# unum-cloud/usearch

Measured on NVIDIA H100. Metric: QPS @ recall@10>=0.95, higher is better.
Workload: dtype f32

## Files before the change

### include/usearch_b200.h

```cpp
#ifndef USEARCH_B200_H
#define USEARCH_B200_H

#include <stdbool.h>
#include <stddef.h>
#include <stdint.h>

#ifdef __cplusplus
extern "C" {
#endif


typedef void* usearch_index_t;
typedef uint64_t usearch_key_t;
typedef float usearch_distance_t;
typedef char const* usearch_error_t;
typedef usearch_distance_t (*usearch_metric_t)(void const*, void const*);

typedef enum usearch_metric_kind_t {
    usearch_metric_unknown_k = 0,
    usearch_metric_cos_k = 1,
    usearch_metric_ip_k = 2,
    usearch_metric_l2sq_k = 3,
    usearch_metric_haversine_k = 4,
    usearch_metric_divergence_k = 5,
// ... 72 lines not shown
                           size_t* counts, usearch_error_t* error);


void usearch_add(usearch_index_t index, usearch_key_t key, void const* vector, usearch_scalar_kind_t vector_kind, usearch_error_t* error);
bool usearch_contains(usearch_index_t index, usearch_key_t key, usearch_error_t* error);
size_t usearch_count(usearch_index_t index, usearch_key_t key, usearch_error_t* error);
size_t usearch_get(usearch_index_t index, usearch_key_t key, size_t count, void* vector, usearch_scalar_kind_t vector_kind, usearch_error_t* error);
size_t usearch_remove(usearch_index_t index, usearch_key_t key, usearch_error_t* error);
size_t usearch_rename(usearch_index_t index, usearch_key_t from, usearch_key_t to, usearch_error_t* error);
usearch_distance_t usearch_distance(void const* vector_first, void const* vector_second, usearch_scalar_kind_t scalar_kind,
                                    size_t dimensions, usearch_metric_kind_t metric_kind, usearch_error_t* error);
void usearch_exact_search(void const* dataset, size_t dataset_size, size_t dataset_stride, void const* queries,
                          size_t queries_size, size_t queries_stride, usearch_scalar_kind_t scalar_kind, size_t dimensions,
                          usearch_metric_kind_t metric_kind, size_t count, size_t threads, usearch_key_t* keys,
                          size_t keys_stride, usearch_distance_t* distances, size_t distances_stride,
                          usearch_error_t* error);
void usearch_clear(usearch_index_t index, usearch_error_t* error);

void usearch_b200_add_many(usearch_index_t index, usearch_key_t const* keys, void const* vectors, size_t count,
                           size_t vectors_stride, usearch_scalar_kind_t vector_kind, usearch_error_t* error);
void usearch_b200_add_many_device(usearch_index_t index, usearch_key_t const* keys, void const* vectors, size_t count,
                                  size_t vectors_stride, usearch_scalar_kind_t vector_kind, usearch_error_t* error);

size_t usearch_b200_remove_many(usearch_index_t index, usearch_key_t const* keys, size_t count, bool compact,
                                size_t* pruned_edges, usearch_error_t* error);
size_t usearch_b200_count_many(usearch_index_t index, usearch_key_t const* keys, size_t count, size_t* counts,
                               usearch_error_t* error);
void usearch_b200_change_reuse_removed(usearch_index_t index, bool reuse, usearch_error_t* error);
bool usearch_b200_reuse_removed(usearch_index_t index);

size_t usearch_b200_join(usearch_index_t a, usearch_index_t b, size_t max_proposals, bool exact, usearch_key_t* a_keys_out,
                         usearch_key_t* b_keys_out, size_t capacity, size_t* stats4_out, usearch_error_t* error);
void usearch_b200_last_join_ms(usearch_index_t index, float* out3);
void usearch_b200_pairwise_distances(usearch_index_t index, usearch_key_t const* left_keys, usearch_key_t const* right_keys, size_t n,
                                     usearch_distance_t* out, usearch_error_t* error);


void usearch_b200_shards_unique_id(void* unique_id128, usearch_error_t* error);
void usearch_b200_shards_join(usearch_index_t index, int rank, int world, void const* unique_id128, usearch_error_t* error);
size_t usearch_b200_sharded_search_many(usearch_index_t index, void const* queries, size_t queries_count, size_t queries_stride,
                                        usearch_scalar_kind_t query_kind, size_t count, usearch_key_t* keys,
                                        usearch_distance_t* distances, size_t* counts, usearch_error_t* error);
void usearch_b200_sharded_search_many_device(usearch_index_t index, void const* queries, size_t queries_count,
                                             size_t queries_stride, size_t count, usearch_key_t* keys,
                                             usearch_distance_t* distances, uint32_t* counts, uint32_t* computed_distances,
                                             uint32_t* visited_members, void* cuda_stream, usearch_error_t* error);
size_t usearch_b200_shards_payload_bytes(size_t queries_count, size_t count);
void usearch_b200_merge_topk(void const* payloads, int world, size_t queries_count, size_t count, usearch_key_t* keys,
                             usearch_distance_t* distances, uint32_t* counts, usearch_error_t* error);


void usearch_b200_search_many_device(usearch_index_t index, void const* queries, size_t queries_count,
                                     size_t queries_stride, size_t count, usearch_key_t* keys,
                                     usearch_distance_t* distances, uint32_t* counts, uint32_t* computed_distances,
                                     uint32_t* visited_members, void* cuda_stream, usearch_error_t* error);

void usearch_b200_search_many_enqueue(usearch_index_t index, void const* queries, size_t queries_count,
                                      size_t queries_stride, size_t count, usearch_key_t* keys,
                                      usearch_distance_t* distances, uint32_t* counts, uint32_t* computed_distances,
                                      uint32_t* visited_members, void* cuda_stream, usearch_error_t* error);
void usearch_b200_search_many_finish(usearch_index_t index, usearch_error_t* error);

size_t usearch_b200_search_many_stats(usearch_index_t index, void const* queries, size_t queries_count,
                                      size_t queries_stride, usearch_scalar_kind_t query_kind, size_t count,
                                      usearch_key_t* keys, usearch_distance_t* distances, size_t* counts,
                                      uint64_t* computed_distances, uint64_t* visited_members, usearch_error_t* error);

size_t usearch_b200_filtered_search_many(usearch_index_t index, void const* queries, size_t queries_count,
                                         size_t queries_stride, usearch_scalar_kind_t query_kind, size_t count,
                                         usearch_key_t const* allowed_keys, size_t allowed_count, usearch_key_t* keys,
                                         usearch_distance_t* distances, size_t* counts, uint64_t* computed_distances,
                                         uint64_t* visited_members, usearch_error_t* error);

void usearch_b200_cluster_many(usearch_index_t index, void const* queries, size_t queries_count, size_t queries_stride,
                               usearch_scalar_kind_t query_kind, size_t level, usearch_key_t* keys,
                               usearch_distance_t* distances, uint64_t* computed_distances, uint64_t* visited_members,
                               usearch_error_t* error);

size_t usearch_b200_exact_search_many(usearch_index_t index, void const* queries, size_t queries_count,
                                      size_t queries_stride, usearch_scalar_kind_t query_kind, size_t count,
                                      usearch_key_t* keys, usearch_distance_t* distances, size_t* counts,
                                      usearch_error_t* error);

void usearch_b200_profile_phases(usearch_index_t index, int enable, uint64_t* counters16);
int usearch_b200_tune(usearch_index_t index, char const* knob, int value);
int usearch_b200_launch_plan(usearch_index_t index, size_t count, uint64_t* out16, usearch_error_t* error);
int usearch_b200_device(usearch_index_t index);
uint64_t usearch_b200_kernel_launches(usearch_index_t index);
float usearch_b200_last_kernel_ms(usearch_index_t index);
size_t usearch_b200_bytes_per_vector(usearch_index_t index);
size_t usearch_b200_max_level(usearch_index_t index);

#ifdef __cplusplus
}
#endif
#endif
```

### usearch_b200/csrc/c_abi.cu

```cuda
#include <sys/mman.h>
#include <sys/stat.h>
#include <fcntl.h>
#include <unistd.h>

#include <cstdio>
#include <algorithm>
#include <cstring>
#include <new>
#include <utility>
#include <vector>

#include "../../include/usearch_b200.h"
#include "frozen_index.h"

using namespace usearch_b200;

namespace {

uint32_t metric_to_char(usearch_metric_kind_t kind) {
    switch (kind) {
    case usearch_metric_ip_k: return METRIC_IP;
    case usearch_metric_l2sq_k: return METRIC_L2SQ;
    case usearch_metric_cos_k: return METRIC_COS;
    case usearch_metric_haversine_k: return 'h';
// ... 474 lines not shown
    if (!m || !s) return set_error(error, "Unknown metric kind!");
    set_error(error, exact_search_free(dataset, dataset_size, dataset_stride, queries, queries_size, queries_stride, s, dimensions, m, count,
                                       keys, keys_stride, distances, distances_stride));
}

void usearch_b200_cluster_many(usearch_index_t index, void const* queries, size_t queries_count, size_t queries_stride,
                               usearch_scalar_kind_t query_kind, size_t level, usearch_key_t* keys, usearch_distance_t* distances,
                               uint64_t* computed_distances, uint64_t* visited_members, usearch_error_t* error) {
    frozen_index_t* ix = as_index(index);
    uint32_t qs = scalar_to_char(query_kind);
    if (!qs) return set_error(error, "Unknown scalar kind!");
    set_error(error, search_host_guarded(ix, queries, queries_count, queries_stride, qs, 1, keys, 8, distances, 4, nullptr, computed_distances,
                                     visited_members, nullptr, nullptr, 0, false, (int)std::min<size_t>(level, 0x7FFF)));
}

size_t usearch_b200_exact_search_many(usearch_index_t index, void const* queries, size_t queries_count, size_t queries_stride,
                                      usearch_scalar_kind_t query_kind, size_t count, usearch_key_t* keys, usearch_distance_t* distances,
                                      size_t* counts, usearch_error_t* error) {
    frozen_index_t* ix = as_index(index);
    uint32_t qs = scalar_to_char(query_kind);
    if (!qs) { set_error(error, "Unknown scalar kind!"); return 0; }
    if (char const* e = ix->exact_host(queries, queries_count, queries_stride, qs, count, keys, distances, counts)) {
        set_error(error, e);
        return 0;
    }
    size_t total = 0;
    if (counts)
        for (size_t i = 0; i < queries_count; ++i) total += counts[i];
    return total;
}


void usearch_b200_shards_unique_id(void* unique_id128, usearch_error_t* error) { set_error(error, shards_unique_id(unique_id128)); }

void usearch_b200_shards_join(usearch_index_t index, int rank, int world, void const* unique_id128, usearch_error_t* error) {
    frozen_index_t* ix = as_index(index);
    std::lock_guard<std::mutex> lock(ix->mutex);
    set_error(error, ix->join_shards(rank, world, unique_id128));
}

size_t usearch_b200_sharded_search_many(usearch_index_t index, void const* queries, size_t queries_count, size_t queries_stride,
                                        usearch_scalar_kind_t query_kind, size_t count, usearch_key_t* keys,
                                        usearch_distance_t* distances, size_t* counts, usearch_error_t* error) {
    frozen_index_t* ix = as_index(index);
    uint32_t qs = scalar_to_char(query_kind);
    if (!qs) { set_error(error, "Unknown scalar kind!"); return 0; }
    if (char const* e = ix->sharded_search_host(queries, queries_count, queries_stride, qs, count, keys, distances, counts)) {
        set_error(error, e);
        return 0;
    }
    size_t total = 0;
    if (counts)
        for (size_t i = 0; i < queries_count; ++i) total += counts[i];
    return total;
}

void usearch_b200_sharded_search_many_device(usearch_index_t index, void const* queries, size_t queries_count, size_t queries_stride,
                                             size_t count, usearch_key_t* keys, usearch_distance_t* distances, uint32_t* counts,
                                             uint32_t* computed_distances, uint32_t* visited_members, void* cuda_stream,
                                             usearch_error_t* error) {
    frozen_index_t* ix = as_index(index);
    std::lock_guard<std::mutex> lock(ix->mutex);
    if (char const* e = ix->ensure_context()) return set_error(error, e);
    cudaStream_t s = cuda_stream ? static_cast<cudaStream_t>(cuda_stream) : ix->stream;
    char const* e = ix->sharded_search_device(queries, queries_count, queries_stride, count, keys, distances, counts,
                                              computed_distances, visited_members, s);
    if (!e && !cuda_stream && cudaStreamSynchronize(s) != cudaSuccess) e = "CUDA failure: synchronize";
    set_error(error, e);
}

size_t usearch_b200_shards_payload_bytes(size_t queries_count, size_t count) { return shards_payload_bytes(queries_count, count); }

void usearch_b200_merge_topk(void const* payloads, int world, size_t queries_count, size_t count, usearch_key_t* keys,
                             usearch_distance_t* distances, uint32_t* counts, usearch_error_t* error) {
    set_error(error, shards_merge_host(payloads, world, queries_count, count, keys, distances, counts));
}

void usearch_clear(usearch_index_t index, usearch_error_t*) {
    frozen_index_t* ix = as_index(index);
    std::lock_guard<std::mutex> lock(ix->mutex);
    ix->release_device();
}

void usearch_b200_profile_phases(usearch_index_t index, int enable, uint64_t* counters16) {
    frozen_index_t* ix = as_index(index);
    std::lock_guard<std::mutex> lock(ix->mutex);
    if (counters16) {
        std::memset(counters16, 0, 128);
        if (ix->phase_cycles.ptr) cudaMemcpy(counters16, ix->phase_cycles.ptr, 128, cudaMemcpyDeviceToHost);
    }
    ix->profile_phases = enable != 0;
    if (ix->profile_phases && !ix->phase_cycles.reserve(16)) cudaMemset(ix->phase_cycles.ptr, 0, 128);
}

int usearch_b200_tune(usearch_index_t index, char const* knob, int value) {
    frozen_index_t* ix = as_index(index);
    std::lock_guard<std::mutex> lock(ix->mutex);
    if (!std::strcmp(knob, "stage_sets")) ix->tune.stage_sets = value;
    else if (!std::strcmp(knob, "warps_per_sm")) ix->tune.warps_per_sm = value;
    else if (!std::strcmp(knob, "prefilter")) ix->tune.prefilter = value;
    else if (!std::strcmp(knob, "heap_head")) ix->tune.heap_head = value;
    else return -1;
    return 0;
}

int usearch_b200_launch_plan(usearch_index_t index, size_t count, uint64_t* out16, usearch_error_t* error) {
    frozen_index_t* ix = as_index(index);
    std::lock_guard<std::mutex> lock(ix->mutex);
    char const* e = ix->ensure_context();
    if (!e && (!ix->loaded || ix->d.n == 0)) e = "An empty index has no launch plan";
    launch_plan_t pl;
    if (!e) e = ix->plan((uint32_t)count, 0, pl);
    set_error(error, e);
    if (e) return -1;
    uint64_t const visits = pl.visited_bitmap_words ? (pl.visit_log_cap ? 2u : 1u) : 0u;
    uint64_t const v[16] = {pl.stage_sets, pl.warps_per_sm_target, (uint64_t)pl.blocks, pl.smem_per_warp,
                            pl.heap_smem_cap, pl.heap_spill_cap, visits, pl.visited_cap,
                            pl.code_pass, pl.code_smem_stride, pl.qsplit_len, pl.prefilter ? 1u : 0u,
                            pl.off_heap - pl.off_stage};
    std::memcpy(out16, v, sizeof(v));
    return 0;
}

int usearch_b200_device(usearch_index_t index) { return as_index(index)->device; }
uint64_t usearch_b200_kernel_launches(usearch_index_t index) { return as_index(index)->kernel_launches; }
float usearch_b200_last_kernel_ms(usearch_index_t index) { return as_index(index)->last_kernel_ms; }
size_t usearch_b200_bytes_per_vector(usearch_index_t index) { return as_index(index)->d.bytes_per_vector; }
size_t usearch_b200_max_level(usearch_index_t index) { return (size_t)as_index(index)->d.max_level; }

}
```

### usearch_b200/csrc/device_index.h

```cpp
#pragma once
#include <cstddef>
#include <cstdint>

namespace usearch_b200 {

struct pf_record_t;

constexpr uint32_t EMPTY_SLOT = 0xFFFFFFFFu;
constexpr uint32_t SNAN_BITS = 0x7FA00000u;

enum : uint32_t {
    METRIC_IP = 'i', METRIC_COS = 'c', METRIC_L2SQ = 'e', METRIC_HAMMING = 'b',
    METRIC_TANIMOTO = 't', METRIC_SORENSEN = 's', METRIC_JACCARD = 'j',
};
enum : uint32_t { SCALAR_B1 = 1, SCALAR_BF16 = 4, SCALAR_F64 = 10, SCALAR_F32 = 11, SCALAR_F16 = 12, SCALAR_I8 = 23 };

struct device_index_t {
    uint8_t const* vectors = nullptr;
    uint64_t const* keys = nullptr;
    uint32_t const* nbr0 = nullptr;
    uint32_t const* upper_base = nullptr;
    uint32_t const* upper = nullptr;
    uint32_t const* deleted_bits = nullptr;
    float const* norms = nullptr;
    int8_t const* codes = nullptr;
    pf_record_t const* shadow = nullptr;
    uint32_t code_stride = 0;
    uint64_t vec_stride = 0;
    uint32_t n = 0;
    uint32_t m0 = 0, m0_stride = 0;
    uint32_t m = 0, m_stride = 0;
    uint32_t entry_slot = 0;
    int32_t max_level = 0;
    uint32_t dims = 0;
    uint32_t bytes_per_vector = 0;
    uint32_t chunks16 = 0;
    uint32_t metric = 0, scalar = 0;
};

struct cand_t {
    float d;
    uint32_t s;
};

enum : uint32_t { STATUS_OK = 0, STATUS_VISITED_OVERFLOW = 1, STATUS_HEAP_OVERFLOW = 2 };

struct search_args_t {
    uint8_t const* queries = nullptr;
    uint64_t query_stride = 0;
    uint32_t nq = 0;
    uint32_t const* query_list = nullptr;
    uint32_t k = 0, ef = 0;
    int32_t cluster_end_level = -1;
    uint8_t const* task_levels = nullptr;
    uint32_t* out_slots = nullptr;
    uint64_t* out_keys = nullptr;
    float* out_dists = nullptr;
    uint32_t* out_counts = nullptr;
    uint32_t* out_computed = nullptr;
    uint32_t* out_visited = nullptr;
    uint32_t* status = nullptr;
    uint32_t const* allow_bits = nullptr;
    uint32_t* work_counter = nullptr;
    uint32_t* visited = nullptr;
    uint32_t visited_cap = 0;
    uint32_t visited_bitmap_words = 0;
    uint32_t* visit_log = nullptr;
    uint32_t visit_log_cap = 0;
    cand_t* heap_spill = nullptr;
    uint32_t heap_spill_cap = 0;
    uint32_t heap_smem_cap = 0;
    uint32_t smem_per_warp = 0, off_top_d = 0, off_top_s = 0, off_cand_s = 0, off_cand_d = 0, off_heap = 0;
    uint32_t off_bars = 0, off_stage = 0, stage_stride = 0;
    uint32_t stage_sets = 1;
    uint32_t prefilter = 0, code_pass = 0, code_smem_stride = 0, off_surv_b2 = 0;
    uint32_t off_qsplit = 0, qsplit_len = 0;
    unsigned long long* phase_cycles = nullptr;
};

}
```

### usearch_b200/csrc/frozen_index.cu

```cuda
#include "cuda_check.h"
#include "f64_casts.h"
#include "frozen_index.h"
#include "prefilter_bound.h"

#include <algorithm>
#include <cmath>
#include <cstdlib>
#include <cstring>

namespace usearch_b200 {

namespace {

uint64_t rd_u64(uint8_t const* p) { uint64_t v; std::memcpy(&v, p, 8); return v; }
uint32_t rd_u32(uint8_t const* p) { uint32_t v; std::memcpy(&v, p, 4); return v; }
int16_t rd_i16(uint8_t const* p) { int16_t v; std::memcpy(&v, p, 2); return v; }
uint32_t ceil2(uint64_t v) { uint64_t r = 1; while (r < v) r <<= 1; return (uint32_t)std::min<uint64_t>(r, 1ull << 31); }
uint32_t round_up(uint32_t v, uint32_t m) { return (v + m - 1) / m * m; }


}

int default_device() {
    if (char const* dev = std::getenv("USEARCH_B200_DEVICE")) return std::atoi(dev);
// ... 470 lines not shown
    if (char const* e = work_counter.reserve(2)) return e;
    size_t const words = warps * pl.visited_words_per_warp();
    bool const grown = words > visited.capacity;
    if (char const* e = visited.reserve(words)) return e;
    if (grown) visited_zeroed_words = 0;
    if (pl.visit_log_cap) {
        if (char const* e = visit_log.reserve(warps * pl.visit_log_cap)) return e;
        if (visited_zeroed_words < words) {
            if (cudaMemsetAsync(visited.ptr, 0, words * 4, s) != cudaSuccess) return "CUDA failure: memset";
            visited_zeroed_words = words;
        }
    } else
        visited_zeroed_words = 0;
    if (char const* e = heap_spill.reserve(warps * pl.heap_spill_cap)) return e;
    a = search_args_t{};
    a.ef = pl.ef;
    a.work_counter = work_counter.ptr;
    a.visited = visited.ptr;
    a.visited_cap = pl.visited_cap;
    a.visited_bitmap_words = pl.visited_bitmap_words;
    a.visit_log = pl.visit_log_cap ? visit_log.ptr : nullptr;
    a.visit_log_cap = pl.visit_log_cap;
    a.heap_spill = heap_spill.ptr;
    a.heap_spill_cap = pl.heap_spill_cap;
    a.heap_smem_cap = pl.heap_smem_cap;
    a.smem_per_warp = pl.smem_per_warp;
    a.off_top_d = pl.off_top_d; a.off_top_s = pl.off_top_s; a.off_cand_s = pl.off_cand_s;
    a.off_cand_d = pl.off_cand_d; a.off_heap = pl.off_heap;
    a.off_bars = pl.off_bars; a.off_stage = pl.off_stage; a.stage_stride = pl.stage_stride;
    a.stage_sets = pl.stage_sets;
    a.prefilter = pl.prefilter ? 1u : 0u;
    a.code_pass = pl.code_pass;
    a.code_smem_stride = pl.code_smem_stride;
    a.off_surv_b2 = pl.off_surv_b2;
    a.off_qsplit = pl.off_qsplit; a.qsplit_len = pl.qsplit_len;
    return nullptr;
}

char const* frozen_index_t::search_device(void const* d_queries, size_t nq, size_t stride, size_t k, uint64_t* d_keys,
                                          float* d_dists, uint32_t* d_counts, uint32_t* d_computed, uint32_t* d_cycles,
                                          cudaStream_t s, bool defer) {
    if (nq == 0 || k == 0) return nullptr;
    if (nq > 0x7FFFFFFFull) return "Too many queries in one batch";
    if (char const* e = ensure_context()) return e;
    if (!loaded || d.n == 0) {
        CU(search_fill_empty(d_keys, d_dists, d_counts, d_computed, d_cycles, nq, k, s));
        return nullptr;
    }
    launch_plan_t pl;
    if (char const* e = plan((uint32_t)k, 0, pl)) return e;
    int const wpb = search_warps_per_block();
    int blocks = (int)std::min<size_t>((size_t)pl.blocks, (nq + wpb - 1) / wpb);
    size_t warps = (size_t)blocks * wpb;

    if (char const* e = h_status.reserve(nq)) return e;
    uint32_t* status_ptr = nullptr;
    if (defer) {
        if (pending_free.empty()) pending_free.emplace_back(new device_buffer_t<uint32_t>());
        device_buffer_t<uint32_t>* buf = pending_free.back();
        pending_free.pop_back();
        if (char const* e = buf->reserve(nq)) { pending_free.push_back(buf); return e; }
        pending.push_back(pending_search_t{buf, search_args_t{}, pl.maxed, s});
        status_ptr = buf->ptr;
    } else {
        if (char const* e = status.reserve(nq)) return e;
        status_ptr = status.ptr;
    }
    search_args_t a;
    if (char const* e = prepare_launch(pl, warps, a, s)) return e;
    a.queries = static_cast<uint8_t const*>(d_queries);
    a.query_stride = stride;
    a.nq = (uint32_t)nq;
    a.k = (uint32_t)k;
    a.out_keys = d_keys;
    a.out_dists = d_dists;
    a.out_counts = d_counts;
    a.out_computed = d_computed;
    a.out_visited = d_cycles;
    a.status = status_ptr;
    a.allow_bits = active_allow_bits;
    a.cluster_end_level = active_cluster_end_level;

    if (profile_phases) {
        if (char const* e = phase_cycles.reserve(16)) return e;
        a.phase_cycles = phase_cycles.ptr;
    }
    CU(cudaMemsetAsync(work_counter.ptr, 0, 8, s));
    CU(cudaEventRecord(ev_begin, s));
    CU(search_launch(d, a, blocks, pl.smem_per_block, s));
    CU(cudaEventRecord(ev_end, s));
    kernel_launches += 1;
    if (defer) {
        pending.back().args = a;
        return nullptr;
    }
    CU(cudaMemcpyAsync(h_status.ptr, status.ptr, nq * 4, cudaMemcpyDeviceToHost, s));
    CU(cudaStreamSynchronize(s));
    CU(cudaEventElapsedTime(&last_kernel_ms, ev_begin, ev_end));
    return retry_overflowed(a, pl.maxed, s);
}

char const* frozen_index_t::search_finish() {
    char const* first_error = nullptr;
    for (pending_search_t& p : pending) {
        char const* e = cuda_error(cudaStreamSynchronize(p.stream));
        if (!e) e = h_status.reserve(p.args.nq);
        if (!e) e = cuda_error(cudaMemcpy(h_status.ptr, p.status->ptr, (size_t)p.args.nq * 4, cudaMemcpyDeviceToHost));
        if (!e) e = retry_overflowed(p.args, p.maxed, p.stream);
        if (e && !first_error) first_error = e;
        pending_free.push_back(p.status);
    }
    pending.clear();
    if (ev_begin && ev_end && !first_error) cudaEventElapsedTime(&last_kernel_ms, ev_begin, ev_end);
    return first_error;
}

char const* frozen_index_t::retry_overflowed(search_args_t const& a, bool maxed, cudaStream_t s) {
    size_t const nq = a.nq, k = a.k;
    int const wpb = search_warps_per_block();
    std::vector<uint32_t> failed;
    for (size_t i = 0; i < nq; ++i)
        if (h_status.ptr[i] != STATUS_OK) failed.push_back((uint32_t)i);
    uint64_t scale = 1;
    while (!failed.empty()) {
        if (maxed) return "Search scratch overflow that full-size scratch could not fix";
        scale *= 8;
        launch_plan_t rp;
        if (char const* e = plan((uint32_t)k, (uint32_t)std::min<uint64_t>(scale, 1u << 30), rp)) return e;
        maxed = rp.maxed;
        size_t const bytes_per_warp = (size_t)rp.visited_words_per_warp() * 4 + (size_t)rp.heap_spill_cap * 8;
        size_t max_warps = std::max<size_t>(wpb, ((size_t)2 << 30) / bytes_per_warp / wpb * wpb);
        int rblocks = (int)std::min<size_t>({(size_t)rp.blocks, (failed.size() + wpb - 1) / wpb, max_warps / wpb});
        rblocks = std::max(rblocks, 1);
        size_t rwarps = (size_t)rblocks * wpb;
        if (char const* e = retry_list.reserve(failed.size())) return e;
        CU(cudaMemcpyAsync(retry_list.ptr, failed.data(), failed.size() * 4, cudaMemcpyHostToDevice, s));
        search_args_t r;
        if (char const* e = prepare_launch(rp, rwarps, r, s)) return e;
        r.queries = a.queries; r.query_stride = a.query_stride; r.k = a.k;
        r.out_keys = a.out_keys; r.out_dists = a.out_dists; r.out_counts = a.out_counts;
        r.out_computed = a.out_computed; r.out_visited = a.out_visited; r.status = a.status;
        r.allow_bits = a.allow_bits; r.cluster_end_level = a.cluster_end_level; r.phase_cycles = a.phase_cycles;
        r.nq = (uint32_t)failed.size();
        r.query_list = retry_list.ptr;
        CU(cudaMemsetAsync(work_counter.ptr, 0, 8, s));
        CU(search_launch(d, r, rblocks, rp.smem_per_block, s));
        kernel_launches += 1;
        CU(cudaMemcpyAsync(h_status.ptr, a.status, nq * 4, cudaMemcpyDeviceToHost, s));
        CU(cudaStreamSynchronize(s));
        std::vector<uint32_t> still;
        for (uint32_t qi : failed)
            if (h_status.ptr[qi] != STATUS_OK) still.push_back(qi);
        failed.swap(still);
    }
    return nullptr;
}


namespace {

uint16_t f32_to_f16_rn(float f) {
    uint32_t x;
    std::memcpy(&x, &f, 4);
    uint32_t sign = (x >> 16) & 0x8000u;
    uint32_t mant = x & 0x7FFFFFu;
    int32_t exp = (int32_t)((x >> 23) & 0xFF);
    if (exp == 255) return (uint16_t)(sign | 0x7C00u | (mant ? 0x200u | (mant >> 13) : 0));
// ... 419 lines not shown
```

### usearch_b200/csrc/search_kernel.cu

```cuda
#include <cuda_runtime.h>

#include <cstdlib>

#include "device_index.h"
#include "metrics.cuh"
#include "warp_primitives.cuh"

namespace usearch_b200 {

constexpr int THREADS = 32;
constexpr int LOADS_IN_FLIGHT = 8;
constexpr int BATCH_LOADS = 4;

__device__ __forceinline__ uint32_t hash_slot(uint32_t s) { return s * 0x9E3779B1u; }


struct heap_t {
    uint32_t smem_addr;
    cand_t* spill;
    uint32_t smem_cap;
    static __device__ __forceinline__ cand_t lds(uint32_t addr) {
        cand_t c;
        asm volatile("ld.shared.v2.b32 {%0, %1}, [%2];" : "=f"(c.d), "=r"(c.s) : "r"(addr));
        return c;
// ... 310 lines not shown
        if ((uint32_t)lane < ncand) w.cand_d[lane] = M::finalize(w.cand_d[lane], qc, n0);
        if ((uint32_t)lane + 32 < ncand) w.cand_d[lane + 32] = M::finalize(w.cand_d[lane + 32], qc, n1);
        for (uint32_t c = 64 + lane; c < ncand; c += 32) w.cand_d[c] = M::finalize(w.cand_d[c], qc, __ldg(ix.norms + w.cand_s[c]));
        __syncwarp();
    }
}

__device__ __forceinline__ pf_record_t ldg_record(pf_record_t const* p) {
    float4 const v = __ldg(reinterpret_cast<float4 const*>(p));
    return pf_record_t{v.x, v.y, v.z, v.w};
}

__device__ __forceinline__ double warp_sum_f64(double v) {
#pragma unroll
    for (int o = 16; o; o >>= 1) v += __shfl_xor_sync(0xffffffffu, v, o);
    return v;
}

__device__ __forceinline__ double warp_max_f64(double v) {
#pragma unroll
    for (int o = 16; o; o >>= 1) v = fmax(v, __shfl_xor_sync(0xffffffffu, v, o));
    return v;
}

__device__ __forceinline__ uint32_t qsplit_word_place(uint32_t word) { return (word & ~7u) + (word & 3u) * 2u + ((word >> 2) & 1u); }

__device__ __forceinline__ pf_query_split_t split_query(float const* qa, uint32_t n, uint8_t* q1, uint8_t* q2, uint32_t len,
                                                        int lane) {
    double mx1 = 0.0;
    bool finite = true;
    for (uint32_t i = (uint32_t)lane; i < n; i += 32) {
        double const x = fabs((double)qa[i]);
        finite = finite && x < INFINITY;
        mx1 = fmax(mx1, x);
    }
    mx1 = warp_max_f64(mx1);
    finite = __all_sync(0xffffffffu, finite);
    float const sa1 = pf_scale(mx1);
    bool const usable = finite && sa1 > 0.0f;
    double mx2 = 0.0;
    int8_t c1, c2;
    if (usable)
        for (uint32_t i = (uint32_t)lane; i < n; i += 32) mx2 = fmax(mx2, fabs(pf_split_step((double)qa[i], sa1, c1)));
    mx2 = warp_max_f64(mx2);
    float const sa2 = usable ? pf_scale(mx2) : 0.0f;
    double e2 = 0.0;
    for (uint32_t wd = (uint32_t)lane; wd < len / 4; wd += 32) {
        uint32_t p1 = 0, p2 = 0;
#pragma unroll
        for (uint32_t b = 0; b < 4; ++b) {
            uint32_t const i = 4 * wd + b;
            c1 = c2 = 0;
            if (usable && i < n) {
                double const r2 = pf_split_step(pf_split_step((double)qa[i], sa1, c1), sa2, c2);
                e2 += r2 * r2;
            }
            p1 |= (uint32_t)(uint8_t)c1 << (8 * b);
            p2 |= (uint32_t)(uint8_t)c2 << (8 * b);
        }
        reinterpret_cast<uint32_t*>(q1)[qsplit_word_place(wd)] = p1;
        reinterpret_cast<uint32_t*>(q2)[qsplit_word_place(wd)] = p2;
    }
    e2 = warp_sum_f64(e2);
    __syncwarp();
    return usable ? pf_query_split_t{sa1, sa2, pf_round_up_norm(e2)} : pf_query_split_t{0.0f, 0.0f, INFINITY};
}

__device__ __forceinline__ void ldmatrix_x4(uint32_t addr, uint32_t& r0, uint32_t& r1, uint32_t& r2, uint32_t& r3) {
    asm volatile("ldmatrix.sync.aligned.m8n8.x4.shared.b16 {%0, %1, %2, %3}, [%4];"
                 : "=r"(r0), "=r"(r1), "=r"(r2), "=r"(r3)
                 : "r"(addr));
}

__device__ __forceinline__ void imma_16832(int (&c)[4], uint32_t a0, uint32_t a1, uint32_t a2, uint32_t a3, uint32_t b0, uint32_t b1) {
    asm volatile("mma.sync.aligned.m16n8k32.row.col.s32.s8.s8.s32 {%0,%1,%2,%3}, {%4,%5,%6,%7}, {%8,%9}, {%0,%1,%2,%3};"
                 : "+r"(c[0]), "+r"(c[1]), "+r"(c[2]), "+r"(c[3])
                 : "r"(a0), "r"(a1), "r"(a2), "r"(a3), "r"(b0), "r"(b1));
}

template <class M>
__device__ __forceinline__ uint32_t measure_prefiltered(device_index_t const& ix, search_args_t const& a, warp_ctx_t& w,
                                                     typename M::qconst_t qc, pf_query_bound_t const& qb,
                                                     pf_query_split_t const& sp, float radius, uint32_t ncand, int lane) {
    constexpr uint32_t MAX_TILES = 4;
    uint8_t* const smem = reinterpret_cast<uint8_t*>(w.q4);
    float* const surv_b2 = reinterpret_cast<float*>(smem + a.off_surv_b2);
    uint32_t const cs = ix.code_stride, scs = a.code_smem_stride, ksteps = a.qsplit_len / 32;
    uint32_t const bar = w.bars_addr;
    uint32_t const g = (uint32_t)lane >> 2, sub = (uint32_t)lane & 3;
    uint32_t const b_addr = smem_u32(smem + a.off_qsplit) + g * a.qsplit_len + 8u * sub;
    uint32_t const a_addr = w.stage_addr + ((uint32_t)lane & 7u) * scs + (((uint32_t)lane >> 3) & 1u) * 8u * scs + ((uint32_t)lane >> 4) * 16u;
    double const sa1 = (double)sp.sa1, sa2 = (double)sp.sa2;
    uint32_t ns = 0;
    for (uint32_t base = 0; base < ncand; base += a.code_pass) {
        uint32_t const cnt = min(a.code_pass, ncand - base);
        if (lane == 0) mbar_expect_tx(bar, cnt * cs);
        __syncwarp();
        pf_record_t r0{}, r1{};
        uint32_t s0 = 0, s1 = 0;
        if ((uint32_t)lane < cnt) {
            s0 = w.cand_s[base + lane];
            bulk_copy_g2s(w.stage_addr + lane * scs, ix.codes + (size_t)s0 * cs, cs, bar);
            r0 = ldg_record(ix.shadow + s0);
        }
        if ((uint32_t)lane + 32 < cnt) {
            s1 = w.cand_s[base + lane + 32];
            bulk_copy_g2s(w.stage_addr + (lane + 32) * scs, ix.codes + (size_t)s1 * cs, cs, bar);
            r1 = ldg_record(ix.shadow + s1);
        }
        if (a.phase_cycles) {
            long long const t = clock64();
            mbar_wait(bar, w.phase & 1u);
            w.t_code += (uint32_t)(clock64() - t);
        } else
            mbar_wait(bar, w.phase & 1u);
        w.phase ^= 1u;
        long long const t_dot = a.phase_cycles ? clock64() : 0;
        uint32_t const ntiles = (cnt + 15) / 16;
        int acc[2][MAX_TILES][4] = {};
        uint32_t fa[2][MAX_TILES][4], fb[2][2];
        auto load = [&](uint32_t k, uint32_t(&A)[MAX_TILES][4], uint32_t(&B)[2]) {
            B[0] = B[1] = 0u;
            if (lane < 8) asm volatile("ld.shared.v2.b32 {%0, %1}, [%2];" : "=r"(B[0]), "=r"(B[1]) : "r"(b_addr + 32u * k));
#pragma unroll
            for (uint32_t t = 0; t < MAX_TILES; ++t)
                if (t < ntiles) ldmatrix_x4(a_addr + t * 16u * scs + 32u * k, A[t][0], A[t][1], A[t][2], A[t][3]);
        };
        auto mma = [&](int (&C)[MAX_TILES][4], uint32_t const(&A)[MAX_TILES][4], uint32_t const(&B)[2]) {
#pragma unroll
            for (uint32_t t = 0; t < MAX_TILES; ++t)
                if (t < ntiles) imma_16832(C[t], A[t][0], A[t][1], A[t][2], A[t][3], B[0], B[1]);
        };
        load(0, fa[0], fb[0]);
        uint32_t k = 0;
        for (; k + 2 <= ksteps; k += 2) {
            load(k + 1, fa[1], fb[1]);
            mma(acc[0], fa[0], fb[0]);
            if (k + 2 < ksteps) load(k + 2, fa[0], fb[0]);
            mma(acc[1], fa[1], fb[1]);
        }
        if (k < ksteps) mma(acc[0], fa[0], fb[0]);
#pragma unroll
        for (uint32_t t = 0; t < MAX_TILES; ++t) {
            uint32_t const i = 16u * t + g;
            int const d1 = acc[0][t][0] + acc[1][t][0], d2 = acc[0][t][1] + acc[1][t][1];
            int const d1h = acc[0][t][2] + acc[1][t][2], d2h = acc[0][t][3] + acc[1][t][3];
            if (sub == 0 && i < cnt) w.cand_d[base + i] = __double2float_rn(sa1 * (double)d1 + sa2 * (double)d2);
            if (sub == 0 && i + 8 < cnt) w.cand_d[base + i + 8] = __double2float_rn(sa1 * (double)d1h + sa2 * (double)d2h);
        }
        __syncwarp();
        long long const t_bound = a.phase_cycles ? clock64() : 0;
        if (a.phase_cycles) w.t_dot += (uint32_t)(t_bound - t_dot);
        uint32_t const lt = (1u << lane) - 1u;
#pragma unroll
        for (int h = 0; h < 2; ++h) {
            uint32_t const i = (uint32_t)lane + 32u * (uint32_t)h, c = base + i;
            if (32u * (uint32_t)h >= cnt) break;
            pf_record_t const r = h ? r1 : r0;
            bool keep = false;
            if (i < cnt) keep = !(M::pf_lower(w.cand_d[c], r, qb) >= (double)radius);
            uint32_t const bal = __ballot_sync(0xffffffffu, keep);
            if (keep) {
                w.cand_s[ns + __popc(bal & lt)] = h ? s1 : s0;
                surv_b2[ns + __popc(bal & lt)] = r.b2;
            }
            ns += __popc(bal);
        }
        __syncwarp();
        if (a.phase_cycles) w.t_bound += (uint32_t)(clock64() - t_bound);
    }
    if (ns) {
        measure_staged<M>(ix, a, w, qc, ns, lane, w.cand_s, w.cand_d);
        __syncwarp();
        if constexpr (M::NORMS) {
            for (uint32_t j = lane; j < ns; j += 32) w.cand_d[j] = M::finalize(w.cand_d[j], qc, surv_b2[j]);
            __syncwarp();
        }
    }
    return ns;
}

__device__ __forceinline__ bool slot_allowed(device_index_t const& ix, search_args_t const& a, uint32_t s) {
    if (ix.deleted_bits && ((ix.deleted_bits[s >> 5] >> (s & 31)) & 1u)) return false;
    if (a.allow_bits && !((a.allow_bits[s >> 5] >> (s & 31)) & 1u)) return false;
    return true;
}


template <class M, bool STAGED, bool INSERT>
__device__ __forceinline__ void search_one(device_index_t const& ix, search_args_t const& a, uint32_t qi, uint32_t out_row,
                                           int const bl_arg, warp_ctx_t& w, heap_t const& heap, uint32_t* visited, int lane) {
    uint32_t const k = a.k, ef = a.ef;
    constexpr bool insert = INSERT;
    int const bl = INSERT ? bl_arg : 0;
    uint32_t const width = bl == 0 ? ix.m0 : ix.m;
    auto row_of = [&](uint32_t slot) -> uint32_t const* {
        if (bl == 0) return ix.nbr0 + (size_t)slot * ix.m0_stride;
        uint32_t const ub = __ldg(ix.upper_base + slot);
        return ix.upper + ((size_t)ub + (uint32_t)(bl - 1)) * ix.m_stride;
    };
    uint32_t top_size = 0, heap_size = 0, computed = 0, cycles = 0, status = STATUS_OK;
    uint32_t visited_total = 0;
    bool log_overflow_out = false;
    bool const prof = a.phase_cycles != nullptr;
    uint32_t pc0 = 0, pc1 = 0, pc2 = 0, pc4 = 0, pc5 = 0, n_push = 0, max_heap = 0, n_pref = 0, n_surv = 0;
    constexpr bool PF = prefilter_of<M>::value && STAGED && !INSERT;
    long long tp = prof ? clock64() : 0;
    w.t_wait = 0;
    w.t_code = 0;
    w.t_dot = 0;
    w.t_bound = 0;
#define PHASE(acc)                                  \
    if (prof) {                                     \
        long long now_ = clock64();                 \
        acc += (uint32_t)(now_ - tp);               \
        tp = now_;                                  \
    }
    float* const top_d = w.top_d;
    uint32_t* const top_s = w.top_s;
    bool const topreg = ef <= 32u * TOP_E;
    float rtd[TOP_E];
    uint32_t rts[TOP_E];
#pragma unroll
    for (int c = 0; c < TOP_E; ++c) { rtd[c] = 0.f; rts[c] = 0u; }
    uint32_t* const cand_s = w.cand_s;
    float* const cand_d = w.cand_d;

    if (ix.n != 0 && k != 0) {
        {
            uint8_t const* src = a.queries + (size_t)qi * a.query_stride;
            uint32_t const bpv = ix.bytes_per_vector;
            bool wide = ((reinterpret_cast<size_t>(src) | a.query_stride) & 15) == 0 && a.query_stride >= (uint64_t)ix.chunks16 * 16;
            if (wide) {
                for (uint32_t j = lane; j < ix.chunks16; j += 32) w.q4[j] = reinterpret_cast<uint4 const*>(src)[j];
            } else {
                uint8_t* dst = reinterpret_cast<uint8_t*>(w.q4);
                for (uint32_t b = lane; b < ix.chunks16 * 16; b += 32) dst[b] = b < bpv ? src[b] : (uint8_t)0;
            }
        }
        bool const bitmap = a.visited_bitmap_words != 0;
        bool const logged = bitmap && a.visit_log != nullptr;
        uint32_t* const vlog = logged ? a.visit_log + (size_t)blockIdx.x * a.visit_log_cap : nullptr;
        bool log_overflow = false;
        if (!logged) {
            uint32_t const fill = bitmap ? 0u : EMPTY_SLOT;
            uint4 const word = make_uint4(fill, fill, fill, fill);
            uint4* v4 = reinterpret_cast<uint4*>(visited);
            uint32_t const n4 = (bitmap ? a.visited_bitmap_words : a.visited_cap) / 4;
            for (uint32_t j = lane; j < n4; j += 32) v4[j] = word;
        }
        __threadfence_block();
        __syncwarp();
        typename M::qconst_t qc = M::prepare(w.q4, ix.chunks16, lane);
        pf_query_split_t pf_sp{0.f, 0.f, INFINITY};
        pf_query_bound_t pf_qb{};
        if constexpr (PF) {
            if (a.prefilter) {
                float const a2 = cos_f32_t::self_dot(w.q4, ix.chunks16, lane);
                uint8_t* const q1 = reinterpret_cast<uint8_t*>(w.q4) + a.off_qsplit;
                pf_sp = split_query(reinterpret_cast<float const*>(w.q4), ix.dims, q1, q1 + a.qsplit_len, a.qsplit_len, lane);
                pf_qb = pf_query_bound(a2, ix.dims, pf_sp.rho_a);
            }
        }
        uint32_t const vmask = a.visited_cap - 1;
        uint32_t visited_count = 0;

        uint32_t closest = ix.entry_slot;
        if (lane == 0) cand_s[0] = closest;
        __syncwarp();
        measure_list<M, STAGED>(ix, a, w, qc, 1, lane);
        computed += 1;
        float closest_d = cand_d[0];
        __syncwarp();
        bool const cluster = a.cluster_end_level >= 0;
        int const end_level = cluster ? a.cluster_end_level : bl;
        for (int level = ix.max_level; level > end_level; --level) {
            bool changed;
            do {
                changed = false;
                uint32_t const ubase = ix.upper_base[closest];
                uint32_t const* row = ix.upper + ((size_t)ubase + (uint32_t)(level - 1)) * ix.m_stride;
                uint32_t n = 0;
                for (uint32_t b = 0; b < ix.m; b += 32) {
                    uint32_t i = b + lane;
                    uint32_t s = (i < ix.m && ubase != EMPTY_SLOT) ? row[i] : EMPTY_SLOT;
                    bool valid = s != EMPTY_SLOT;
                    uint32_t bal = __ballot_sync(0xffffffffu, valid);
                    if (valid) cand_s[n + __popc(bal & ((1u << lane) - 1))] = s;
                    n += __popc(bal);
                }
                __syncwarp();
                measure_list<M, STAGED>(ix, a, w, qc, n, lane);
                computed += n;
                for (uint32_t b = 0; b < n; b += 32) {
                    uint32_t i = b + lane;
                    float d = i < n ? cand_d[i] : 0.f;
                    bool better = i < n && d < closest_d;
                    float best = better ? d : __int_as_float(0x7f800000);
                    uint32_t best_i = better ? i : 0xFFFFFFFFu;
#pragma unroll
                    for (int o = 16; o; o >>= 1) {
                        float od = __shfl_xor_sync(0xffffffffu, best, o);
                        uint32_t oi = __shfl_xor_sync(0xffffffffu, best_i, o);
                        if (oi != 0xFFFFFFFFu && (best_i == 0xFFFFFFFFu || od < best || (od == best && oi < best_i))) {
                            best = od;
                            best_i = oi;
                        }
                    }
                    if (best_i != 0xFFFFFFFFu) {
                        closest_d = best;
                        closest = cand_s[best_i];
                        changed = true;
                    }
                }
                __syncwarp();
                cycles += 1;
            } while (changed);
        }

        if (lane == 0) cand_s[0] = closest;
        __syncwarp();
        measure_list<M, STAGED>(ix, a, w, qc, 1, lane);
        computed += 1;
        float radius = cand_d[0];
        __syncwarp();
        if (lane == 0 && !cluster) {
            heap.set_root(cand_t{radius, closest});
            if (bitmap) atomicOr(&visited[closest >> 5], 1u << (closest & 31));
            else atomicCAS(&visited[hash_slot(closest) & vmask], EMPTY_SLOT, closest);
            if (logged) vlog[0] = closest;
        }
        heap_size = cluster ? 0 : 1;
        visited_count = cluster ? 0 : 1;
        uint32_t pre_node = EMPTY_SLOT, pre_s0 = EMPTY_SLOT, pre_s1 = EMPTY_SLOT;
        constexpr bool WIDE = !STAGED;
        uint32_t pre_s2 = EMPTY_SLOT, pre_s3 = EMPTY_SLOT;
        PHASE(pc0)
        {
            bool allowed = cluster || (insert ? closest != qi : slot_allowed(ix, a, closest));
            if (allowed) {
                if (topreg) {
                    if (lane == 0) { rtd[0] = radius; rts[0] = closest; }
                } else if (lane == 0) { top_d[0] = radius; top_s[0] = closest; }
                top_size = 1;
            }
        }
        __syncwarp();

        while (heap_size) {
            cand_t cur = heap.root();
            if (cur.d > radius && top_size == ef) break;
            uint32_t const* row = row_of(cur.s);
            uint32_t s0, s1, s2 = EMPTY_SLOT, s3 = EMPTY_SLOT;
            if (cur.s == pre_node) {
                s0 = pre_s0;
                s1 = pre_s1;
                if constexpr (WIDE) { s2 = pre_s2; s3 = pre_s3; }
            } else {
                s0 = lane < (int)width ? __ldg(row + lane) : EMPTY_SLOT;
                s1 = lane + 32 < (int)width ? __ldg(row + lane + 32) : EMPTY_SLOT;
                if constexpr (WIDE) {
                    s2 = lane + 64 < (int)width ? __ldg(row + lane + 64) : EMPTY_SLOT;
                    s3 = lane + 96 < (int)width ? __ldg(row + lane + 96) : EMPTY_SLOT;
                }
            }
            __syncwarp();
            uint32_t o0 = 0xFFFFFFFFu, o1 = 0xFFFFFFFFu, o2 = 0xFFFFFFFFu, o3 = 0xFFFFFFFFu;
            if (bitmap) {
                if (s0 != EMPTY_SLOT) o0 = atomicOr(&visited[s0 >> 5], 1u << (s0 & 31));
                if (s1 != EMPTY_SLOT) o1 = atomicOr(&visited[s1 >> 5], 1u << (s1 & 31));
                if constexpr (WIDE) {
                    if (s2 != EMPTY_SLOT) o2 = atomicOr(&visited[s2 >> 5], 1u << (s2 & 31));
                    if (s3 != EMPTY_SLOT) o3 = atomicOr(&visited[s3 >> 5], 1u << (s3 & 31));
                }
            }
            if (!heap.template pop_warp<PF ? 16 : 8>(heap_size, lane)) {
                if (lane == 0) heap.pop(heap_size);
            }
            heap_size -= 1;
            cycles += 1;
            __syncwarp();
            if (heap_size) {
                pre_node = heap.root().s;
                uint32_t const* next_row = row_of(pre_node);
                pre_s0 = lane < (int)width ? __ldg(next_row + lane) : EMPTY_SLOT;
                pre_s1 = lane + 32 < (int)width ? __ldg(next_row + lane + 32) : EMPTY_SLOT;
                if constexpr (WIDE) {
                    pre_s2 = lane + 64 < (int)width ? __ldg(next_row + lane + 64) : EMPTY_SLOT;
                    pre_s3 = lane + 96 < (int)width ? __ldg(next_row + lane + 96) : EMPTY_SLOT;
                }
            } else
                pre_node = EMPTY_SLOT;
            PHASE(pc1)

            uint32_t ncand = 0;
            if (bitmap) {
                bool f0 = s0 != EMPTY_SLOT && !((o0 >> (s0 & 31)) & 1u);
                bool f1 = s1 != EMPTY_SLOT && !((o1 >> (s1 & 31)) & 1u);
                uint32_t bal0 = __ballot_sync(0xffffffffu, f0), bal1 = __ballot_sync(0xffffffffu, f1);
                uint32_t const lt = (1u << lane) - 1;
                if (f0) cand_s[__popc(bal0 & lt)] = s0;
// ... 456 lines not shown
```

### usearch_b200/index.py

```python
from __future__ import annotations

import ctypes as C
import os
from dataclasses import dataclass
from typing import Dict, Optional, Union

import numpy as np

HERE = os.path.dirname(os.path.abspath(__file__))
LIB_PATH = os.path.join(HERE, "libusearch_b200.so")

METRIC_KIND = {"cos": 1, "ip": 2, "l2sq": 3, "haversine": 4, "divergence": 5, "pearson": 6, "jaccard": 7,
               "hamming": 8, "tanimoto": 9, "sorensen": 10}
SCALAR_KIND = {"f32": 1, "f64": 2, "f16": 3, "i8": 4, "b1": 5, "bf16": 6}
_NP_TO_SCALAR = {np.dtype(np.float32): "f32", np.dtype(np.float64): "f64", np.dtype(np.float16): "f16",
                 np.dtype(np.int8): "i8", np.dtype(np.uint8): "b1"}
_BITS = {"f32": 32, "f64": 64, "f16": 16, "bf16": 16, "i8": 8, "b1": 1}


class _InitOptions(C.Structure):
    _fields_ = [("metric_kind", C.c_int), ("metric", C.c_void_p), ("quantization", C.c_int),
                ("dimensions", C.c_size_t), ("connectivity", C.c_size_t), ("expansion_add", C.c_size_t),
                ("expansion_search", C.c_size_t), ("multi", C.c_bool)]

# ... 459 lines not shown
            keys.ctypes.data_as(C.c_void_p), distances.ctypes.data_as(C.c_void_p),
            computed.ctypes.data_as(C.c_void_p) if stats else None, visited.ctypes.data_as(C.c_void_p) if stats else None,
            C.byref(err))
        _raise(err)
        if stats:
            self.last_computed, self.last_visited = computed, visited
        return keys, distances

    def search(self, vectors: np.ndarray, count: int = 10, *, stats: bool = False, threads: int = 0, exact: bool = False,
               log=False, progress=None, _allowed: Optional[np.ndarray] = None) -> Union[Matches, BatchMatches]:
        vectors = np.asarray(vectors)
        single = vectors.ndim == 1
        if single:
            vectors = vectors[None, :]
        if vectors.ndim != 2:
            raise ValueError("Expects a matrix or a vector")
        if not vectors.flags.c_contiguous and vectors.strides[1] != vectors.itemsize:
            vectors = np.ascontiguousarray(vectors)
        kind = self._kind_of(vectors)
        expect_cols = (self.ndim * _BITS[kind] + 7) // 8 // vectors.itemsize if kind != "b1" else (self.ndim + 7) // 8
        if vectors.shape[1] != expect_cols:
            raise ValueError("The number of columns must match the dimensionality of the index")
        nq = vectors.shape[0]
        keys = np.zeros((nq, count), dtype=np.uint64)
        distances = np.zeros((nq, count), dtype=np.float32)
        counts = np.zeros(nq, dtype=np.uint64)
        err = C.c_char_p()
        vm = cd = 0
        if exact:
            self._lib.usearch_b200_exact_search_many(
                self._h, vectors.ctypes.data_as(C.c_void_p), nq, vectors.strides[0], SCALAR_KIND[kind], count,
                keys.ctypes.data_as(C.c_void_p), distances.ctypes.data_as(C.c_void_p),
                counts.ctypes.data_as(C.c_void_p), C.byref(err))
            _raise(err)
        elif _allowed is not None:
            computed = np.zeros(nq, dtype=np.uint64)
            visited = np.zeros(nq, dtype=np.uint64)
            self._lib.usearch_b200_filtered_search_many(
                self._h, vectors.ctypes.data_as(C.c_void_p), nq, vectors.strides[0], SCALAR_KIND[kind], count,
                _allowed.ctypes.data_as(C.c_void_p), _allowed.size, keys.ctypes.data_as(C.c_void_p),
                distances.ctypes.data_as(C.c_void_p), counts.ctypes.data_as(C.c_void_p),
                computed.ctypes.data_as(C.c_void_p), visited.ctypes.data_as(C.c_void_p), C.byref(err))
            _raise(err)
            self.last_computed, self.last_visited = computed, visited
            vm, cd = int(visited.sum()), int(computed.sum())
        elif stats:
            computed = np.zeros(nq, dtype=np.uint64)
            visited = np.zeros(nq, dtype=np.uint64)
            self._lib.usearch_b200_search_many_stats(
                self._h, vectors.ctypes.data_as(C.c_void_p), nq, vectors.strides[0], SCALAR_KIND[kind], count,
                keys.ctypes.data_as(C.c_void_p), distances.ctypes.data_as(C.c_void_p),
                counts.ctypes.data_as(C.c_void_p), computed.ctypes.data_as(C.c_void_p),
                visited.ctypes.data_as(C.c_void_p), C.byref(err))
            _raise(err)
            self.last_computed, self.last_visited = computed, visited
            vm, cd = int(visited.sum()), int(computed.sum())
        else:
            self._lib.usearch_search_many(
                self._h, vectors.ctypes.data_as(C.c_void_p), nq, vectors.strides[0], SCALAR_KIND[kind], count,
                keys.ctypes.data_as(C.c_void_p), keys.strides[0], distances.ctypes.data_as(C.c_void_p),
                distances.strides[0], counts.ctypes.data_as(C.c_void_p), C.byref(err))
            _raise(err)
        if single:
            n = int(counts[0])
            return Matches(keys[0, :n], distances[0, :n], vm, cd)
        return BatchMatches(keys, distances, counts, vm, cd)

    def tune(self, **knobs: int) -> None:
        for name, value in knobs.items():
            if self._lib.usearch_b200_tune(self._h, name.encode(), int(value)) != 0:
                raise ValueError(f"unknown knob {name}")

    def launch_plan(self, count: int = 10) -> dict:
        out = np.zeros(16, dtype=np.uint64)
        err = C.c_char_p()
        self._lib.usearch_b200_launch_plan(self._h, int(count), out.ctypes.data_as(C.c_void_p), C.byref(err))
        _raise(err)
        plan = dict(zip(LAUNCH_PLAN_FIELDS, (int(v) for v in out)))
        plan["visits"] = _VISITS[plan["visits"]]
        plan["prefilter"] = bool(plan["prefilter"])
        return plan

    def profile_phases(self, enable: bool = True) -> dict:
        out = np.zeros(16, dtype=np.uint64)
        self._lib.usearch_b200_profile_phases(self._h, int(enable), out.ctypes.data_as(C.c_void_p))
        names = ["setup_descent", "heap_pop", "row_visited", "vector_wait", "distance_math", "accept", "output"]
        q = max(int(out[7]), 1)
        return {"queries": int(out[7]), **{n: float(out[i]) / q for i, n in enumerate(names)},
                "pushes": float(out[8]) / q, "avg_max_heap": float(out[9]) / q, "max_heap": int(out[10]),
                "prefiltered": float(out[11]) / q, "survivors": float(out[12]) / q, "code_wait": float(out[13]) / q,
                "prefilter_dot": float(out[14]) / q, "prefilter_bound": float(out[15]) / q,
                "survivor_math": float(out[4] - out[14] - out[15]) / q}

    def join_shards(self, rank: int, world: int, unique_id: bytes) -> None:
        err = C.c_char_p()
        buf = (C.c_char * 128).from_buffer_copy(unique_id)
        self._lib.usearch_b200_shards_join(self._h, rank, world, buf, C.byref(err))
        _raise(err)

    def sharded_search(self, vectors: np.ndarray, count: int = 10) -> BatchMatches:
        vectors = np.ascontiguousarray(vectors)
        if vectors.ndim == 1:
            vectors = vectors[None, :]
        kind = self._kind_of(vectors)
        nq = vectors.shape[0]
        keys = np.zeros((nq, count), dtype=np.uint64)
        distances = np.zeros((nq, count), dtype=np.float32)
        counts = np.zeros(nq, dtype=np.uint64)
        err = C.c_char_p()
        self._lib.usearch_b200_sharded_search_many(self._h, vectors.ctypes.data_as(C.c_void_p), nq, vectors.strides[0],
                                                   SCALAR_KIND[kind], count, keys.ctypes.data_as(C.c_void_p),
                                                   distances.ctypes.data_as(C.c_void_p), counts.ctypes.data_as(C.c_void_p),
                                                   C.byref(err))
        _raise(err)
        return BatchMatches(keys, distances, counts)

    def sharded_search_device(self, queries_ptr: int, nq: int, stride: int, count: int, keys_ptr: int, distances_ptr: int,
                              counts_ptr: int, computed_ptr: int = 0, visited_ptr: int = 0, stream: int = 0) -> None:
        err = C.c_char_p()
        self._lib.usearch_b200_sharded_search_many_device(self._h, queries_ptr, nq, stride, count, keys_ptr, distances_ptr,
                                                          counts_ptr, computed_ptr or None, visited_ptr or None,
                                                          stream or None, C.byref(err))
        _raise(err)

    def search_enqueue(self, queries_ptr: int, nq: int, stride: int, count: int, keys_ptr: int, distances_ptr: int,
                       counts_ptr: int, computed_ptr: int = 0, visited_ptr: int = 0, stream: int = 0) -> None:
        err = C.c_char_p()
        self._lib.usearch_b200_search_many_enqueue(self._h, queries_ptr, nq, stride, count, keys_ptr, distances_ptr,
                                                   counts_ptr, computed_ptr or None, visited_ptr or None,
                                                   stream or None, C.byref(err))
        _raise(err)

    def search_finish(self) -> None:
        err = C.c_char_p()
        self._lib.usearch_b200_search_many_finish(self._h, C.byref(err))
        _raise(err)

    def search_device(self, queries_ptr: int, nq: int, stride: int, count: int, keys_ptr: int, distances_ptr: int,
                      counts_ptr: int, computed_ptr: int = 0, visited_ptr: int = 0, stream: int = 0) -> None:
        err = C.c_char_p()
        self._lib.usearch_b200_search_many_device(self._h, queries_ptr, nq, stride, count, keys_ptr, distances_ptr,
                                                  counts_ptr, computed_ptr or None, visited_ptr or None,
                                                  stream or None, C.byref(err))
        _raise(err)


def exact_search(dataset: np.ndarray, queries: np.ndarray, count: int = 10, *, metric: str = "cos",
                 dtype: Optional[str] = None) -> BatchMatches:
    lib = load_library()
    dataset = np.ascontiguousarray(dataset)
    queries = np.ascontiguousarray(queries)
    if queries.ndim == 1:
        queries = queries[None, :]
    kind = dtype or ("bf16" if dataset.dtype == np.uint16 else _NP_TO_SCALAR[dataset.dtype])
    dims = dataset.shape[1] * 8 if kind == "b1" else dataset.shape[1]
    nq = queries.shape[0]
    keys = np.zeros((nq, count), dtype=np.uint64)
    distances = np.zeros((nq, count), dtype=np.float32)
    err = C.c_char_p()
    lib.usearch_exact_search(dataset.ctypes.data_as(C.c_void_p), dataset.shape[0], dataset.strides[0],
                             queries.ctypes.data_as(C.c_void_p), nq, queries.strides[0], SCALAR_KIND[kind], dims,
                             METRIC_KIND[metric], count, 0, keys.ctypes.data_as(C.c_void_p), keys.strides[0],
                             distances.ctypes.data_as(C.c_void_p), distances.strides[0], C.byref(err))
    _raise(err)
    return BatchMatches(keys, distances, np.full(nq, count, dtype=np.uint64))


def shards_unique_id() -> bytes:
    lib = load_library()
    buf = (C.c_char * 128)()
    err = C.c_char_p()
    lib.usearch_b200_shards_unique_id(buf, C.byref(err))
    _raise(err)
    return bytes(buf)
# ... 22 lines not shown
```

Measured before the change: 333,900.

## Apply int8 prefilter during upper-level descent and loop prefilter MMA over tile pairs

In the greedy upper-level descent, the PF kernel variant now sends neighbour lists through the int8 tensor-core prefilter, bounded by the current closest distance, so fewer full-precision distances are computed. The prefilter MMA is restructured to process candidates in pairs of 16-row tiles with a 4-deep k pipeline, which lifts the old 4-tile cap and lets it handle longer lists. A 17th profiling counter records descent rows. The risk is prefilter overhead on short descent lists, plus the chance of pruning the true closest node if the bound is loose.

```diff
diff --git a/include/usearch_b200.h b/include/usearch_b200.h
--- a/include/usearch_b200.h
+++ b/include/usearch_b200.h
@@ -178,7 +178,7 @@
                                       usearch_key_t* keys, usearch_distance_t* distances, size_t* counts,
                                       usearch_error_t* error);
 
-void usearch_b200_profile_phases(usearch_index_t index, int enable, uint64_t* counters16);
+void usearch_b200_profile_phases(usearch_index_t index, int enable, uint64_t* counters17);
 int usearch_b200_tune(usearch_index_t index, char const* knob, int value);
 int usearch_b200_launch_plan(usearch_index_t index, size_t count, uint64_t* out16, usearch_error_t* error);
 int usearch_b200_device(usearch_index_t index);
diff --git a/usearch_b200/csrc/c_abi.cu b/usearch_b200/csrc/c_abi.cu
--- a/usearch_b200/csrc/c_abi.cu
+++ b/usearch_b200/csrc/c_abi.cu
@@ -580,15 +580,16 @@
     ix->release_device();
 }
 
-void usearch_b200_profile_phases(usearch_index_t index, int enable, uint64_t* counters16) {
-    frozen_index_t* ix = as_index(index);
-    std::lock_guard<std::mutex> lock(ix->mutex);
-    if (counters16) {
-        std::memset(counters16, 0, 128);
-        if (ix->phase_cycles.ptr) cudaMemcpy(counters16, ix->phase_cycles.ptr, 128, cudaMemcpyDeviceToHost);
+void usearch_b200_profile_phases(usearch_index_t index, int enable, uint64_t* counters17) {
+    frozen_index_t* ix = as_index(index);
+    std::lock_guard<std::mutex> lock(ix->mutex);
+    size_t const bytes = PHASE_COUNTERS * sizeof(uint64_t);
+    if (counters17) {
+        std::memset(counters17, 0, bytes);
+        if (ix->phase_cycles.ptr) cudaMemcpy(counters17, ix->phase_cycles.ptr, bytes, cudaMemcpyDeviceToHost);
     }
     ix->profile_phases = enable != 0;
-    if (ix->profile_phases && !ix->phase_cycles.reserve(16)) cudaMemset(ix->phase_cycles.ptr, 0, 128);
+    if (ix->profile_phases && !ix->phase_cycles.reserve(PHASE_COUNTERS)) cudaMemset(ix->phase_cycles.ptr, 0, bytes);
 }
 
 int usearch_b200_tune(usearch_index_t index, char const* knob, int value) {
diff --git a/usearch_b200/csrc/device_index.h b/usearch_b200/csrc/device_index.h
--- a/usearch_b200/csrc/device_index.h
+++ b/usearch_b200/csrc/device_index.h
@@ -78,4 +78,6 @@
     unsigned long long* phase_cycles = nullptr;
 };
 
+constexpr uint32_t PHASE_COUNTERS = 17;
+
 }
diff --git a/usearch_b200/csrc/frozen_index.cu b/usearch_b200/csrc/frozen_index.cu
--- a/usearch_b200/csrc/frozen_index.cu
+++ b/usearch_b200/csrc/frozen_index.cu
@@ -576,7 +576,7 @@
     a.cluster_end_level = active_cluster_end_level;
 
     if (profile_phases) {
-        if (char const* e = phase_cycles.reserve(16)) return e;
+        if (char const* e = phase_cycles.reserve(PHASE_COUNTERS)) return e;
         a.phase_cycles = phase_cycles.ptr;
     }
     CU(cudaMemsetAsync(work_counter.ptr, 0, 8, s));
diff --git a/usearch_b200/csrc/search_kernel.cu b/usearch_b200/csrc/search_kernel.cu
--- a/usearch_b200/csrc/search_kernel.cu
+++ b/usearch_b200/csrc/search_kernel.cu
@@ -416,7 +416,7 @@
 __device__ __forceinline__ uint32_t measure_prefiltered(device_index_t const& ix, search_args_t const& a, warp_ctx_t& w,
                                                      typename M::qconst_t qc, pf_query_bound_t const& qb,
                                                      pf_query_split_t const& sp, float radius, uint32_t ncand, int lane) {
-    constexpr uint32_t MAX_TILES = 4;
+    constexpr uint32_t TILES = 2;
     uint8_t* const smem = reinterpret_cast<uint8_t*>(w.q4);
     float* const surv_b2 = reinterpret_cast<float*>(smem + a.off_surv_b2);
     uint32_t const cs = ix.code_stride, scs = a.code_smem_stride, ksteps = a.qsplit_len / 32;
@@ -451,36 +451,40 @@
         w.phase ^= 1u;
         long long const t_dot = a.phase_cycles ? clock64() : 0;
         uint32_t const ntiles = (cnt + 15) / 16;
-        int acc[2][MAX_TILES][4] = {};
-        uint32_t fa[2][MAX_TILES][4], fb[2][2];
-        auto load = [&](uint32_t k, uint32_t(&A)[MAX_TILES][4], uint32_t(&B)[2]) {
-            B[0] = B[1] = 0u;
-            if (lane < 8) asm volatile("ld.shared.v2.b32 {%0, %1}, [%2];" : "=r"(B[0]), "=r"(B[1]) : "r"(b_addr + 32u * k));
-#pragma unroll
-            for (uint32_t t = 0; t < MAX_TILES; ++t)
-                if (t < ntiles) ldmatrix_x4(a_addr + t * 16u * scs + 32u * k, A[t][0], A[t][1], A[t][2], A[t][3]);
-        };
-        auto mma = [&](int (&C)[MAX_TILES][4], uint32_t const(&A)[MAX_TILES][4], uint32_t const(&B)[2]) {
-#pragma unroll
-            for (uint32_t t = 0; t < MAX_TILES; ++t)
-                if (t < ntiles) imma_16832(C[t], A[t][0], A[t][1], A[t][2], A[t][3], B[0], B[1]);
-        };
-        load(0, fa[0], fb[0]);
-        uint32_t k = 0;
-        for (; k + 2 <= ksteps; k += 2) {
-            load(k + 1, fa[1], fb[1]);
-            mma(acc[0], fa[0], fb[0]);
-            if (k + 2 < ksteps) load(k + 2, fa[0], fb[0]);
-            mma(acc[1], fa[1], fb[1]);
-        }
-        if (k < ksteps) mma(acc[0], fa[0], fb[0]);
-#pragma unroll
-        for (uint32_t t = 0; t < MAX_TILES; ++t) {
-            uint32_t const i = 16u * t + g;
-            int const d1 = acc[0][t][0] + acc[1][t][0], d2 = acc[0][t][1] + acc[1][t][1];
-            int const d1h = acc[0][t][2] + acc[1][t][2], d2h = acc[0][t][3] + acc[1][t][3];
-            if (sub == 0 && i < cnt) w.cand_d[base + i] = __double2float_rn(sa1 * (double)d1 + sa2 * (double)d2);
-            if (sub == 0 && i + 8 < cnt) w.cand_d[base + i + 8] = __double2float_rn(sa1 * (double)d1h + sa2 * (double)d2h);
+        for (uint32_t t0 = 0; t0 < ntiles; t0 += TILES) {
+            bool const pair = t0 + 1 < ntiles;
+            int acc[4][TILES][4] = {};
+            uint32_t fa[4][TILES][4], fb[4][2];
+            auto load = [&](uint32_t k, uint32_t(&A)[TILES][4], uint32_t(&B)[2]) {
+                B[0] = B[1] = 0u;
+                if (lane < 8) asm volatile("ld.shared.v2.b32 {%0, %1}, [%2];" : "=r"(B[0]), "=r"(B[1]) : "r"(b_addr + 32u * k));
+                uint32_t const at = a_addr + t0 * 16u * scs + 32u * k;
+                ldmatrix_x4(at, A[0][0], A[0][1], A[0][2], A[0][3]);
+                if (pair) ldmatrix_x4(at + 16u * scs, A[1][0], A[1][1], A[1][2], A[1][3]);
+            };
+            auto mma = [&](int (&C)[TILES][4], uint32_t const(&A)[TILES][4], uint32_t const(&B)[2]) {
+                imma_16832(C[0], A[0][0], A[0][1], A[0][2], A[0][3], B[0], B[1]);
+                if (pair) imma_16832(C[1], A[1][0], A[1][1], A[1][2], A[1][3], B[0], B[1]);
+            };
+            load(0, fa[0], fb[0]);
+            if (1 < ksteps) load(1, fa[1], fb[1]);
+            for (uint32_t k = 0; k < ksteps; k += 4) {
+#pragma unroll
+                for (uint32_t u = 0; u < 4; ++u) {
+                    if (k + u + 2 < ksteps) load(k + u + 2, fa[(u + 2) & 3], fb[(u + 2) & 3]);
+                    if (k + u < ksteps) mma(acc[u], fa[u], fb[u]);
+                }
+            }
+#pragma unroll
+            for (uint32_t t = 0; t < TILES; ++t) {
+                uint32_t const i = 16u * (t0 + t) + g;
+                int const d1 = (acc[0][t][0] + acc[1][t][0]) + (acc[2][t][0] + acc[3][t][0]);
+                int const d2 = (acc[0][t][1] + acc[1][t][1]) + (acc[2][t][1] + acc[3][t][1]);
+                int const d1h = (acc[0][t][2] + acc[1][t][2]) + (acc[2][t][2] + acc[3][t][2]);
+                int const d2h = (acc[0][t][3] + acc[1][t][3]) + (acc[2][t][3] + acc[3][t][3]);
+                if (sub == 0 && i < cnt) w.cand_d[base + i] = __double2float_rn(sa1 * (double)d1 + sa2 * (double)d2);
+                if (sub == 0 && i + 8 < cnt) w.cand_d[base + i + 8] = __double2float_rn(sa1 * (double)d1h + sa2 * (double)d2h);
+            }
         }
         __syncwarp();
         long long const t_bound = a.phase_cycles ? clock64() : 0;
@@ -624,8 +628,15 @@
                     n += __popc(bal);
                 }
                 __syncwarp();
-                measure_list<M, STAGED>(ix, a, w, qc, n, lane);
-                computed += n;
+                if constexpr (PF) {
+                    computed += n;
+                    if (a.prefilter && n) n = measure_prefiltered<M>(ix, a, w, qc, pf_qb, pf_sp, closest_d, n, lane);
+                    else measure_list<M, STAGED>(ix, a, w, qc, n, lane);
+                    if (prof && lane == 0) atomicAdd(a.phase_cycles + 16, (unsigned long long)n);
+                } else {
+                    measure_list<M, STAGED>(ix, a, w, qc, n, lane);
+                    computed += n;
+                }
                 for (uint32_t b = 0; b < n; b += 32) {
                     uint32_t i = b + lane;
                     float d = i < n ? cand_d[i] : 0.f;
@@ -651,6 +662,7 @@
                 cycles += 1;
             } while (changed);
         }
+        if constexpr (PF) { w.t_code = 0; w.t_dot = 0; w.t_bound = 0; }
 
         if (lane == 0) cand_s[0] = closest;
         __syncwarp();
diff --git a/usearch_b200/index.py b/usearch_b200/index.py
--- a/usearch_b200/index.py
+++ b/usearch_b200/index.py
@@ -565,7 +565,7 @@
         return plan
 
     def profile_phases(self, enable: bool = True) -> dict:
-        out = np.zeros(16, dtype=np.uint64)
+        out = np.zeros(17, dtype=np.uint64)
         self._lib.usearch_b200_profile_phases(self._h, int(enable), out.ctypes.data_as(C.c_void_p))
         names = ["setup_descent", "heap_pop", "row_visited", "vector_wait", "distance_math", "accept", "output"]
         q = max(int(out[7]), 1)
@@ -573,6 +573,7 @@
                 "pushes": float(out[8]) / q, "avg_max_heap": float(out[9]) / q, "max_heap": int(out[10]),
                 "prefiltered": float(out[11]) / q, "survivors": float(out[12]) / q, "code_wait": float(out[13]) / q,
                 "prefilter_dot": float(out[14]) / q, "prefilter_bound": float(out[15]) / q,
+                "descent_rows": float(out[16]) / q,
                 "survivor_math": float(out[4] - out[14] - out[15]) / q}
 
     def join_shards(self, rank: int, world: int, unique_id: bytes) -> None:
```

New measurement: 341,900, median of 6. +2.4%, better.
